# ChristophReich1996/Multi-StyleGAN

Measured on AMD Instinct MI355X. Metric: training images/sec (G+D step, 256^2, seq=3x2ch), higher is better.
Workload: dtype bf16

## Files before the change

### include/msg_hip.h

```cpp
#ifndef MSG_HIP_H
#define MSG_HIP_H

#ifdef __cplusplus
extern "C" {
#endif

enum { MSG_OK = 0, MSG_EINVAL = -1, MSG_EUNSUPPORTED = -2, MSG_ELAUNCH = -3 };
enum { MSG_F32 = 0, MSG_BF16 = 1, MSG_F16 = 2, MSG_F64 = 3, MSG_F32_SPLIT = 4 };

#define MSG_ABI_VERSION 5
int msg_abi_version(void);
const char* msg_build_arch(void);
const char* msg_strerror(int code);

int msg_upfirdn2d(const void* x, const float* fir, void* y, int dtype,
                  int major, int in_h, int in_w, int minor, int kh, int kw,
                  int up_x, int up_y, int down_x, int down_y,
                  int pad_x0, int pad_x1, int pad_y0, int pad_y1, void* stream);

int msg_upfirdn2d_pitched(const void* x, const float* fir, void* y, int dtype,
                          int major, int in_h, int in_w, int minor, int in_pitch, int kh, int kw,
                          int up_x, int up_y, int down_x, int down_y,
                          int pad_x0, int pad_x1, int pad_y0, int pad_y1, void* stream);

int msg_upfirdn2d_pitched2(const void* x, const float* fir, void* y, int dtype,
                           int major, int in_h, int in_w, int minor, int in_pitch, int out_pitch, int kh, int kw,
                           int up_x, int up_y, int down_x, int down_y,
                           int pad_x0, int pad_x1, int pad_y0, int pad_y1, void* stream);

int msg_upfirdn2d_separable(const void* x, const float* fir_y, const float* fir_x, void* y, int dtype,
                            int major, int in_h, int in_w, int minor, int kh, int kw,
                            int pad_x0, int pad_x1, int pad_y0, int pad_y1, void* stream);

int msg_upfirdn2d_separable_act(const void* x, const float* fir_y, const float* fir_x, void* y, int dtype,
                                int major, int in_h, int in_w, int minor, int kh, int kw,
                                int pad_x0, int pad_x1, int pad_y0, int pad_y1,
                                const float* act_bias, const float* noise, const float* noise_weight,
                                int noise_batch, float alpha, float scale, void* stream);
int msg_upfirdn2d_separable_act_mask(const void* x, const float* fir_y, const float* fir_x, void* y, int dtype,
                                     int major, int in_h, int in_w, int minor, int kh, int kw,
                                     int pad_x0, int pad_x1, int pad_y0, int pad_y1,
                                     const float* act_bias, const float* noise, const float* noise_weight,
                                     int noise_batch, float alpha, float scale, unsigned char* mask, void* stream);

int msg_fused_bias_act(const void* x, const float* bias, const void* ref, void* y, int dtype,
                       long long size_x, int step_b, int size_b,
                       const float* noise, const float* noise_weight, int noise_batch, int pix,
                       int act, int grad, float alpha, float scale, void* stream);

long long msg_bias_act_backward_workspace(long long size_x, int step_b, int size_b, int has_noise);
int msg_bias_act_backward(const void* gy, const void* out, void* gx, int dtype,
                          long long size_x, int step_b, int size_b,
                          float* grad_bias, const float* noise, float* grad_noise_weight,
                          int noise_batch, int pix, float alpha, float scale,
                          float* ws, long long ws_floats, void* stream);
int msg_channel_sums(const void* x, float* sums, int dtype, long long size_x, int C, float* ws, long long ws_floats,
                     void* stream);
int msg_bias_act_backward_mask(const void* gy, const unsigned char* mask, int tile_m, int tile_n, void* gx, int dtype,
                               long long size_x, int size_b,
                               float* grad_bias, const float* noise, float* grad_noise_weight,
                               int noise_batch, int pix, float alpha, float scale,
                               float* ws, long long ws_floats, void* stream);
int msg_sum_rows(const float* part, float* out, long long rows, int cols, void* stream);
int msg_bias_act_backward_mask_head(const void* gy, const void* ghead, const float* whead, const float* style,
                                    float wscale, int n_head, const unsigned char* mask, int tile_m, int tile_n,
                                    void* gx, int dtype, long long size_x, int size_b,
                                    float* grad_bias, const float* noise, float* grad_noise_weight,
                                    int noise_batch, int pix, float alpha, float scale,
                                    float* ws, long long ws_floats, void* stream);

int msg_conv2d_fprop(const void* x, const void* w, const float* bias, void* y, int dtype,
                     int B, int IH, int IW, int Cx, int Ck, int OH, int OW, int N, int ldy,
                     int kh, int kw, int stride, int pad, int in_up, int pixel_shuffle,
                     long long w_batch_stride, void* stream);
enum { MSG_WGRAD_K_AUTO = -1 };
int msg_conv2d_wgrad(const void* gy, const void* x, float* gw, int dtype,
                     int B, int IH, int IW, int Cx, int I, int OH, int OW, int ldgy, int O, int ldgw,
                     int kh, int kw, int stride, int pad, int pixel_shuffle,
                     int per_sample, int k_chunks, int oi_major, float gain,
                     float* ws, long long ws_floats, void* stream);
long long msg_conv2d_wgrad_workspace(int dtype, int B, int IH, int IW, int Cx, int I, int OH, int OW, int ldgy,
                                     int O, int ldgw, int kh, int kw, int stride, int pad, int pixel_shuffle,
                                     int per_sample, int k_chunks);

int msg_demod_coeff(const float* W, const float* s, float* d, int B, int O, int I, int taps,
                    float scale, float eps, void* stream);
int msg_scale_rows_cols(const float* base, const float* rowscale, const float* colscale, void* out,
                        int dtype, int B, int R, int T, int C, int Ck, float gain, void* stream);
int msg_modulate_weights(const float* base, const float* wsq, const float* style, void* out, float* d_out,
                         int dtype, int B, int R, int O, int T, int C, int Ck, float scale, float eps, void* stream);
int msg_modulate_backward(const float* gwk, const float* W, const float* s, const float* d, float* gW,
                          float* gs_part, int B, int O, int I, int taps, int ldg, int o_group,
                          float scale, void* stream);
int msg_scale_rows_cols2(const float* base, const float* row1, const float* col1, const float* row2, const float* col2,
                         void* out, int dtype, int B, int R, int T, int C, int Ck, float gain, void* stream);
int msg_modulate_backward2(const float* gwk, const float* W, const float* s, const float* d, const float* v,
                           float* gW, float* gs_part, int B, int O, int I, int taps, int ldg, int o_group,
                           float scale, void* stream);

int msg_relayout_weight(const float* w, void* fwd, void* dgrad, float* wsq, int dtype,
                        int O, int I, int T, int Ck, int Ok, int flip, int t_major, float gain, void* stream);

int msg_gather_taps(const void* x, void* y, int dtype, int B, int H, int W, int Cx, int C, int kh, int kw,
                    int pad, int Ko, void* stream);
int msg_fold_taps(const void* g, const void* add, void* gx, int dtype, int B, int H, int W, int Ko, int C, int kh, int kw,
                  int pad, int ldx, int ld_add, void* stream);

int msg_scaled_add(const void* a, const void* b, void* y, int dtype, long long n, float beta, float gain, void* stream);
int msg_rgb_skip_merge(const void* conv, int dtype, int ld, const float* bias, const float* skip, const float* fir,
                       float* out, int B, int C, int H, int W, void* stream);
int msg_rgb_skip_merge_backward(const float* g, void* g_conv, int dtype, int ld, float* g_skip, const float* fir,
                                int B, int C, int H, int W, void* stream);
int msg_gamma_merge(const void* a, const void* b, const float* gamma, void* y, int dtype, long long n, float gain, void* stream);
long long msg_gamma_merge_backward_workspace(void);
int msg_gamma_merge_backward(const void* gy, const void* a, const float* gamma, void* ga, void* gb, float* g_gamma, int dtype,
                             long long n, float gain, float* ws, void* stream);
int msg_scaled_add_rows(const void* a, const void* b, void* y, int dtype, long long rows, int cols,
                        long long lda, long long ldb, long long ldy, float beta, float gain, void* stream);

int msg_softmax_rows(const void* x, void* y, int dtype, long long rows, int cols, void* stream);
int msg_softmax_rows_backward(const void* y, const void* gy, void* gx, int dtype, long long rows, int cols,
                              void* stream);
int msg_softmax_rows_backward2(const void* y, const void* gy, const void* v, void* d_y, void* d_gy, int dtype,
                               long long rows, int cols, void* stream);

int msg_nonlocal_attention_supported(int B, int Nq, int Nk, int dk, int dv);
int msg_nonlocal_attention_fwd(const void* q, const void* k, const void* vt, void* o, float* lse, int dtype,
                               int B, int Nq, int Nk, int dk, int dv, void* stream);
int msg_maxpool2x2_fwd(const void* x, void* y, unsigned short* idx, int dtype, int B, int H, int W, int C, long long ldx,
                       void* stream);
int msg_maxpool2x2_bwd(const void* gy, const unsigned short* idx, void* gx, int dtype, int B, int H, int W, int C,
                       void* stream);
int msg_maxpool2x2_gather(const void* v, const unsigned short* idx, void* out, int dtype, int B, int H, int W, int C,
                          long long ldv, void* stream);

int msg_nonlocal_attention_bwd_splits(int B, int Nq, int Nk);
int msg_nonlocal_attention_bwd(const void* q, const void* qt, const void* k, const void* kt, const void* v,
                               const void* dO, const void* dOt, const void* o, const float* lse, float* delta,
                               void* dq, void* dk_out, void* dv_out, float* workspace, int dtype,
                               int B, int Nq, int Nk, int dk, int dv, void* stream);

int msg_affine_warp(const float* x, float* y, const float* angle_deg, float angle_const, const float* scale_xy,
                    const float* select_u, const float* p, int rot_prob, float cx, float cy, int padding,
                    int align_corners, int B, int C, int H, int W, int backward, void* workspace, void* stream);

long long msg_minibatch_stddev_workspace(int C, int H, int W, int groups, int dtype);
int msg_minibatch_stddev(const void* x, void* y, float* stat, float* workspace, int dtype,
                         int B, int C, int H, int W, int ldx, int ldy, int groups, float alpha, void* stream);
int msg_minibatch_stddev_backward(const void* x, const void* gy, const float* gstat, void* gx, int dtype,
                                  int B, int C, int H, int W, int ldx, int ldgy, int ldgx, int groups,
                                  float alpha, void* stream);

int msg_conv2d_fprop_act(const void* x, const void* w, void* y, int dtype,
                         int B, int IH, int IW, int Cx, int Ck, int OH, int OW, int N, int ldy,
                         int kh, int kw, int stride, int pad, long long w_batch_stride,
                         const float* act_bias, const float* noise, const float* noise_weight,
                         int noise_batch, float alpha, float scale, void* stream);
int msg_conv2d_fprop_act_mask(const void* x, const void* w, void* y, int dtype,
                              int B, int IH, int IW, int Cx, int Ck, int OH, int OW, int N, int ldy,
                              int kh, int kw, int stride, int pad, long long w_batch_stride,
                              const float* act_bias, const float* noise, const float* noise_weight,
                              int noise_batch, float alpha, float scale, unsigned char* mask, void* stream);

int msg_conv2d_fprop_residual(const void* x, const void* w, void* y, int dtype,
                              int B, int IH, int IW, int Cx, int Ck, int OH, int OW, int N, int ldy,
                              int kh, int kw, int stride, int pad, long long w_batch_stride,
                              const void* residual, int res_ld, float gain, void* stream);

int msg_conv2d_fprop_act_backward(const void* x, const void* w, void* y, int dtype,
                                  int B, int IH, int IW, int Cx, int Ck, int OH, int OW, int N, int ldy,
                                  int kh, int kw, int stride, int pad, long long w_batch_stride,
                                  const void* residual, int res_ld,
                                  const unsigned char* sign_mask, int mask_tile_m, int mask_tile_n,
                                  const void* sign_map, int sign_ld, float alpha, float scale,
                                  float* grad_bias, const float* noise, int noise_batch, float* grad_noise_weight,
                                  float* ws, long long ws_floats, void* stream);

int msg_act_pointwise_head(const void* x, const float* bias, const float* w, float* y, int dtype,
                           long long npix, int C, float wscale, float alpha, float scale, void* stream);
long long msg_act_pointwise_head_backward_workspace(long long npix, int C);
int msg_act_pointwise_head_backward(const void* x, const float* bias, const float* w, const float* gy, void* gx,
// ... 111 lines not shown
```

### multi_stylegan_amd/conv_ops.py

```python
import ctypes
import functools
import math
import os
from typing import Optional, Tuple

import torch
from torch.autograd import Function

from . import _lib, weight_images
from ._autograd import _derive
from .weight_images import _k_run, _oi, _round_up
from .weight_images import invalidate_weight_cache


def _vec(dtype) -> int:
    return 8 if dtype == torch.bfloat16 else 4


def _padded_nhwc(b, c, h, w, dtype, device):
    cx = _round_up(c, _vec(dtype))
    buf = torch.empty((b, h, w, cx), dtype=dtype, device=device)
    if cx != c:
        buf[..., c:].zero_()
    return buf.permute(0, 3, 1, 2)[:, :c]
# ... 1250 lines not shown
        if not terms:
            return (None, None, None, None)
        grads = torch.autograd.grad(sum(terms), leaves, allow_unused=True)
    return tuple(gr if w else None for gr, w in zip(grads, want))


class _ModConvGrad(Function):

    @staticmethod
    def forward(ctx, gy, x, weight, style, d, demodulate, upsample, g, scale, need):
        gx, gw, gs, gwk = _modconv_backward(x, weight, style, d, gy, demodulate, upsample, g, scale, need, keep_gwk=True)
        ctx.set_materialize_grads(False)
        ctx.save_for_backward(gy, x, weight, style, d, gwk)
        ctx.cfg = (demodulate, upsample, g, scale)
        return gx, gw, gs

    @staticmethod
    @torch.autograd.function.once_differentiable
    def backward(ctx, a, cot_w, cot_s):
        gy, x, weight, style, d, gwk = ctx.saved_tensors
        demodulate, upsample, g, scale = ctx.cfg
        want = ctx.needs_input_grad[:4]
        _, o, i, kh, kw = weight.shape
        b, t = x.shape[0], kh * kw
        tail = (None,) * 6
        if a is None and cot_w is None and cot_s is None:
            return (None, None, None, None) + tail
        if cot_w is not None or i % 4 or i > 512 or t not in (1, 4, 9) or b > _MODCONV_BWD_BATCH or \
                (cot_s is not None and gwk is None):
            return _modconv_second_order_composite(gy, x, weight, style, demodulate, upsample, a, cot_w, cot_s, want) + tail
        dev = x.device
        w3 = weight.detach().reshape(o, i, t)
        s = style.detach().float().contiguous()
        dd = d if demodulate else None
        ck, okp = _round_up(i, _k_run(gy.dtype)), _round_up(o, _k_run(gy.dtype))
        rows = t * o if upsample else o
        ggy = gx2 = gw3 = gs2 = None
        if a is not None:
            a = a.to(x.dtype)
            if want[0]:
                wk = torch.empty((b, rows, 1 if upsample else t, ck), dtype=x.dtype, device=dev)
                base = weight_images.forward(weight, torch.float32, 1.0, g.kind, modulation=True)[0]
                _scale_rows_cols(base, (d.repeat(1, t) if upsample else d) if demodulate else None, s, wk, scale)
                ggy = _f_image(a, wk, ck, o, i, g)
            if want[2] or want[3]:
                gwk_a, ldg = _g_raw(gy, a, o, i, g, raw=True)
                gw3, gs2 = _fold_weight_gradient(gwk_a, ldg, w3, s, dd, scale, style.dtype)
        if cot_s is not None:
            v = cot_s.detach().float().contiguous()
            if want[0] or want[1]:
                hf = torch.empty((b, rows, 1 if upsample else t, ck), dtype=x.dtype, device=dev)
                hd = torch.empty((b, i, t, okp), dtype=gy.dtype, device=dev)
                base_f = weight_images.forward(weight, torch.float32, 1.0, g.kind, modulation=True)[0]
                base_d = weight_images.dgrad(weight, torch.float32, 1.0, g.kind, modulation=True)[0]
                if demodulate:
                    wsq = weight_images.tap_square_sums(weight, g.kind)
                    ddir = -(scale * scale) * d.pow(3) * linear(s * v, wsq)
                    rows_d, rows_dd = (d.repeat(1, t), ddir.repeat(1, t)) if upsample else (d, ddir)
                    with _lib.on_device(dev):
                        lib, st = _lib.lib(), _lib.stream_of(dev)
                        code = lib.msg_scale_rows_cols2(base_f.data_ptr(), rows_d.contiguous().data_ptr(), v.data_ptr(),
                                                        rows_dd.contiguous().data_ptr(), s.data_ptr(), hf.data_ptr(),
                                                        _lib.dtype_code(hf), b, rows, 1 if upsample else t, i, ck, scale, st)
                        _lib.check(code, "msg_scale_rows_cols2")
                        code = lib.msg_scale_rows_cols2(base_d.data_ptr(), v.data_ptr(), d.data_ptr(), s.data_ptr(),
                                                        ddir.contiguous().data_ptr(), hd.data_ptr(), _lib.dtype_code(hd), b, i, t,
                                                        o, okp, scale, st)
                        _lib.check(code, "msg_scale_rows_cols2")
                else:
                    _scale_rows_cols(base_f, None, v, hf, scale)
                    _scale_rows_cols(base_d, v, None, hd, scale)
                if want[0]:
                    ggy = _f_image(x, hf, ck, o, i, g, residual=None if ggy is None else (ggy, 1.0))
                if want[1]:
                    gx2 = _d_image(gy, hd, okp, o, i, g)
            if want[2] or want[3]:
                gw3b, gs2b = _fold_weight_gradient(gwk, gwk.shape[-1], w3, s, dd, scale, style.dtype, cotangent=v)
                gw3 = gw3b if gw3 is None else gw3 + gw3b
                gs2 = gs2b if gs2 is None else gs2 + gs2b
        gw = gw3.reshape(1, o, i, kh, kw) if (gw3 is not None and want[2]) else None
        return (ggy, gx2, gw, gs2 if want[3] else None) + tail


class _ModulatedConv(Function):

    @staticmethod
    def forward(ctx, x, weight, style, demodulate, upsample, act_bias=None, noise=None, noise_w=None, alpha=0.2,
                act_scale=1.0, fuse_act=False, head_slot=None, input_act=None):
        dev = _lib.require_gpu(x, weight, style)
        ctx.input_act = input_act if input_act is not None and input_act.armed else None
        ctx.head_slot = head_slot
        if head_slot is not None and fuse_act:
            ctx.set_materialize_grads(False)
            head_slot.armed = True
        _, o, i, kh, kw = weight.shape
        b, t = x.shape[0], kh * kw
        scale = math.sqrt(2.0) / math.sqrt(i * t)
        s = style.detach().float().contiguous()
        d = None
        ck = _round_up(i, _k_run(x.dtype))
        kind = "up2" if upsample else "conv"
        base = weight_images.forward(weight, torch.float32, 1.0, kind, modulation=True)[0]
        rows = t * o if upsample else o
        wk = torch.empty((b, rows, 1 if upsample else t, ck), dtype=x.dtype, device=dev)
        if demodulate:
            wsq = weight_images.tap_square_sums(weight, kind)
            d = torch.empty((b, o), dtype=torch.float32, device=dev)
            with _lib.on_device(dev):
                code = _lib.lib().msg_modulate_weights(base.data_ptr(), wsq.data_ptr(), s.data_ptr(), wk.data_ptr(),
                                                       d.data_ptr(), _lib.dtype_code(wk), b, rows, o,
                                                       1 if upsample else t, i, ck, scale, 1e-8, _lib.stream_of(dev))
            _lib.check(code, "msg_modulate_weights")
        else:
            _scale_rows_cols(base, None, s, wk, scale)
        g = Geometry(kind, kh, kw, 1, kh // 2, x.shape[2:], True)
        act = None
        holder = [] if any(ctx.needs_input_grad) else None
        if fuse_act:
            assert not upsample, "the upsampling layers blur before their activation"
            act = (*_act_operands(act_bias, noise, noise_w, (b, o, *g.y_hw)), alpha, act_scale, holder)
        y = _f_image(x, wk, ck, o, i, g, act=act)
        ctx.save_for_backward(x, weight, style, d if d is not None else torch.empty(0, device=dev),
                              y if fuse_act else None, noise if fuse_act else None)
        ctx.cfg = (demodulate, upsample, g, scale)
        ctx.act = (alpha, act_scale, act_bias is not None, noise is not None,
                   None if noise_w is None else noise_w.shape) if fuse_act else None
        ctx.bias_param = act_bias
        ctx.mask = holder[0] if holder else None
        return y

    @staticmethod
    def backward(ctx, gy):
        x, weight, style, d, y_act, noise = ctx.saved_tensors
        demodulate, upsample, g, scale = ctx.cfg
        _, o, i, kh, kw = weight.shape
        b, t = x.shape[0], kh * kw
        need = list(ctx.needs_input_grad)
        need[1], need[2] = _consumed(ctx, 1, 1), _consumed(ctx, 2, 2)
        gb = gnw = None
        slot = ctx.head_slot
        if ctx.act is not None:
            from .op_static.fused_act import FusedLeakyReLUFunctionBackward, act_backward_with_head
            alpha, act_scale, has_bias, has_noise, nw_shape = ctx.act
            head, head_dgrad = slot.take() if slot is not None else (None, None)
            fused = None
            if head is not None:
                fused = act_backward_with_head(gy, head, y_act.shape, noise if has_noise else None,
                                               ctx.bias_param if has_bias else None, has_bias, alpha, act_scale, ctx.mask)
                if fused is None:
                    gh = head_dgrad()
                    gy = gh if gy is None else gy + gh
            if fused is not None:
                gy, gb, gnw = fused
            elif gy is None:
                return (None,) * 13
            else:
                gy, gb, gnw = _derive(FusedLeakyReLUFunctionBackward, gy, y_act, noise if has_noise else None,
                                      ctx.bias_param if has_bias else False, alpha, act_scale, ctx.mask)
            gb = gb if has_bias and need[5] else None
            gnw = gnw.reshape(nw_shape) if has_noise and need[7] else None
        tail = (None, None, gb, None, gnw, None, None, None, None, None)
        if ctx.act is None and slot is not None and slot.armed and need[0] and not torch.is_grad_enabled() and \
                fused_head_ok(gy, weight, b, demodulate, upsample):
            gyc, wt, st = gy, weight, style
            slot.head = (gyc, weight.detach().reshape(o, i).float().contiguous(), style.detach().float().contiguous(), scale)
            slot.dgrad = lambda: _modconv_backward(x, wt, st, d, gyc, demodulate, upsample, g, scale,
                                                   [True, False, False])[0]
            need[0] = False
        fused_ok = i <= 512 and t <= 9
        if torch.is_grad_enabled() and fused_ok and _NATIVE_SECOND_ORDER and b <= _MODCONV_BWD_BATCH and x.is_cuda:
            gx, gw, gs = _derive(_ModConvGrad, gy, x, weight, style, d if demodulate else None, demodulate, upsample, g, scale,
                                            tuple(need[:3]))
            return (gx, gw, gs) + tail
        if torch.is_grad_enabled() or not fused_ok:
            with torch.enable_grad():
                ins = [v for v, n in zip((x, weight, style), need[:3]) if n]
                y2 = _modulated_composite(x, weight, style, demodulate, upsample)
                grads = list(torch.autograd.grad(y2, ins, gy, create_graph=torch.is_grad_enabled(), allow_unused=True))
            out = [grads.pop(0) if n else None for n in need[:3]]
            return (out[0], out[1], out[2]) + tail
        if b > _MODCONV_BWD_BATCH:
            gxs, gws, gss = [], [], []
            for lo in range(0, b, _MODCONV_BWD_BATCH):
                hi = min(b, lo + _MODCONV_BWD_BATCH)
                cgx, cgw, cgs = _modconv_backward(x[lo:hi], weight, style[lo:hi], d[lo:hi] if demodulate else d,
                                                  gy[lo:hi], demodulate, upsample, g, scale, need)
                gxs.append(cgx); gws.append(cgw); gss.append(cgs)
            gx = torch.cat(gxs) if need[0] else None
            gw = torch.stack(gws).sum(dim=0) if gws[0] is not None else None
            gs = torch.cat(gss) if gss[0] is not None else None
            return (gx, gw, gs) + tail
        gx, gw, gs = _modconv_backward(x, weight, style, d, gy, demodulate, upsample, g, scale, need, direct=True,
                                       act_bwd=ctx.input_act)
        return (gx, gw, gs) + tail


def fused_head_ok(gy, weight, b, demodulate, upsample) -> bool:
    _, o, _, kh, kw = weight.shape
    return gy is not None and gy.is_cuda and gy.dtype == torch.bfloat16 and kh == 1 and kw == 1 and o <= 8 and \
        not demodulate and not upsample and b <= _MODCONV_BWD_BATCH and HEAD_GRAD_FUSION


HEAD_GRAD_FUSION = bool(int(os.environ.get("MSG_HEAD_GRAD_FUSION", "1")))

# ... 13 lines not shown
```

### multi_stylegan_amd/csrc/modulate.hip

```cpp
#include "msg_common.h"
#include <stdlib.h>

__device__ __forceinline__ float block_sum_256(float v, float* red ) {
    v = wave_sum(v);
    __syncthreads();
    if ((threadIdx.x & 63) == 0) red[threadIdx.x >> 6] = v;
    __syncthreads();
    return red[0] + red[1] + red[2] + red[3];
}

__global__ __launch_bounds__(256) void demod_coeff_kernel(const float* __restrict__ W, const float* __restrict__ s,
                                                          float* __restrict__ d, int B, int O, int I, int T,
                                                          float scale, float eps) {
    __shared__ float red[4];
    const int o = blockIdx.x;
    const float* wo = W + (size_t)o * I * T;
    for (int b = 0; b < B; ++b) {
        float acc = 0.f;
        for (int i = threadIdx.x; i < I; i += 256) {
            const float sv = s[(size_t)b * I + i];
            float w2 = 0.f;
            for (int t = 0; t < T; ++t) { const float wv = wo[i * T + t]; w2 = fmaf(wv, wv, w2); }
            acc = fmaf(w2, sv * sv, acc);
        }
        const float tot = block_sum_256(acc, red);
        if (threadIdx.x == 0) d[(size_t)b * O + o] = rsqrtf(scale * scale * tot + eps);
    }
}

extern "C" int msg_demod_coeff(const float* W, const float* s, float* d, int B, int O, int I, int taps,
                               float scale, float eps, void* stream) {
    if (B == 0) return MSG_OK;
    if (!W || !s || !d || B < 0 || O <= 0 || I <= 0 || taps <= 0) return MSG_EINVAL;
    hipLaunchKernelGGL(demod_coeff_kernel, dim3(O), dim3(256), 0, (hipStream_t)stream, W, s, d, B, O, I, taps, scale, eps);
    return MSG_CHECK_LAUNCH();
}

template <int VEC>
__device__ __forceinline__ void load_run(const float* __restrict__ src, int c0, int limit, bool aligned, float (&f)[VEC]) {
    if (aligned && c0 + VEC <= limit) {
#pragma unroll
        for (int e = 0; e < VEC; e += 4) {
            const float4 v = *reinterpret_cast<const float4*>(src + c0 + e);
            f[e] = v.x; f[e + 1] = v.y; f[e + 2] = v.z; f[e + 3] = v.w;
        }
    } else {
#pragma unroll
        for (int e = 0; e < VEC; ++e) f[e] = (c0 + e < limit) ? src[c0 + e] : 0.f;
    }
}

constexpr int SRC_ITEMS = 5;
template <typename TO>
__global__ __launch_bounds__(256) void scale_rows_cols_kernel(const float* __restrict__ base,
                                                              const float* __restrict__ rowscale,
                                                              const float* __restrict__ colscale, TO* __restrict__ out,
                                                              int B, int BG, int R, int T, int C, int Ck, float gain) {
    using V = Vec16<TO>;
    constexpr int VEC = V::N;
    const int r = blockIdx.x, b0 = blockIdx.y * BG, b1 = min(B, b0 + BG);
    const int cvecs = Ck / VEC;
    const float* src_row = base + (size_t)r * T * C;
    const int tstep = 256 / cvecs > 0 ? 256 / cvecs : 1;
    const bool al = (C % 4 == 0) && ((((uintptr_t)base | (uintptr_t)colscale) & 15u) == 0);
    for (int cv = threadIdx.x % cvecs; cv < cvecs; cv += 256) {
        const int c0 = cv * VEC;
        const int t0 = threadIdx.x / cvecs;
        for (int tb = t0; tb < T; tb += tstep * SRC_ITEMS) {
            float f[SRC_ITEMS][VEC];
#pragma unroll
            for (int k = 0; k < SRC_ITEMS; ++k) {
                const int t = tb + k * tstep;
                if (t < T) load_run<VEC>(src_row + (size_t)t * C, c0, C, al, f[k]);
                else {
#pragma unroll
                    for (int e = 0; e < VEC; ++e) f[k][e] = 0.f;
                }
            }
            for (int b = b0; b < b1; ++b) {
                const float rs = gain * (rowscale ? rowscale[(size_t)b * R + r] : 1.f);
                float sc[VEC];
                if (colscale) load_run<VEC>(colscale + (size_t)b * C, c0, C, al, sc);
                else {
// ... 49 lines not shown
                                                               TO* __restrict__ out, int B, int BG, int R, int T, int C, int Ck,
                                                               float gain) {
    using V = Vec16<TO>;
    constexpr int VEC = V::N;
    const int r = blockIdx.x, b0 = blockIdx.y * BG, b1 = min(B, b0 + BG);
    const int cvecs = Ck / VEC;
    const float* src_row = base + (size_t)r * T * C;
    const int tstep = 256 / cvecs > 0 ? 256 / cvecs : 1;
    const bool al = (C % 4 == 0) && ((((uintptr_t)base | (uintptr_t)col1 | (uintptr_t)col2) & 15u) == 0);
    for (int cv = threadIdx.x % cvecs; cv < cvecs; cv += 256) {
        const int c0 = cv * VEC;
        const int t0 = threadIdx.x / cvecs;
        for (int tb = t0; tb < T; tb += tstep * SRC_ITEMS) {
            float f[SRC_ITEMS][VEC];
#pragma unroll
            for (int k = 0; k < SRC_ITEMS; ++k) {
                const int t = tb + k * tstep;
                if (t < T) load_run<VEC>(src_row + (size_t)t * C, c0, C, al, f[k]);
                else {
#pragma unroll
                    for (int e = 0; e < VEC; ++e) f[k][e] = 0.f;
                }
            }
            for (int b = b0; b < b1; ++b) {
                const float rs1 = gain * row1[(size_t)b * R + r], rs2 = gain * row2[(size_t)b * R + r];
                float sc[VEC], s2[VEC];
                load_run<VEC>(col1 + (size_t)b * C, c0, C, al, sc);
                load_run<VEC>(col2 + (size_t)b * C, c0, C, al, s2);
#pragma unroll
                for (int e = 0; e < VEC; ++e) sc[e] = fmaf(rs1, sc[e], rs2 * s2[e]);
                TO* dst_row = out + ((size_t)b * R + r) * T * Ck;
#pragma unroll
                for (int k = 0; k < SRC_ITEMS; ++k) {
                    const int t = tb + k * tstep;
                    if (t >= T) break;
                    V o;
                    if constexpr (VEC == 4) {
#pragma unroll
                        for (int e = 0; e < 4; ++e) o.set(e, f[k][e] * sc[e]);
                    } else {
#pragma unroll
                        for (int e = 0; e < 4; ++e) o.set2(e, f[k][2 * e] * sc[2 * e], f[k][2 * e + 1] * sc[2 * e + 1]);
                    }
                    *reinterpret_cast<uint4*>(dst_row + (size_t)t * Ck + c0) = o.raw;
                }
            }
        }
    }
}

extern "C" int msg_scale_rows_cols2(const float* base, const float* row1, const float* col1, const float* row2,
                                    const float* col2, void* out, int dtype, int B, int R, int T, int C, int Ck, float gain,
                                    void* stream) {
    if (B == 0) return MSG_OK;
    if (!base || !row1 || !col1 || !row2 || !col2 || !out || B < 0 || R <= 0 || T <= 0 || C <= 0 || Ck < C) return MSG_EINVAL;
    if (dtype != MSG_F32 && dtype != MSG_BF16) return MSG_EUNSUPPORTED;
    const int vec = dtype == MSG_BF16 ? 8 : 4;
    if (Ck % vec || (((uintptr_t)out) & 15u)) return MSG_EUNSUPPORTED;
    hipStream_t s = (hipStream_t)stream;
    int bg = 1;
    while (bg < 8 && bg * 2 <= B && (long long)R * ((B + 2 * bg - 1) / (2 * bg)) >= 2048) bg *= 2;
    dim3 grid(R, (B + bg - 1) / bg);
    if (dtype == MSG_BF16)
        hipLaunchKernelGGL((scale_rows_cols2_kernel<bf16_t>), grid, dim3(256), 0, s, base, row1, col1, row2, col2,
                           (bf16_t*)out, B, bg, R, T, C, Ck, gain);
    else
        hipLaunchKernelGGL((scale_rows_cols2_kernel<float>), grid, dim3(256), 0, s, base, row1, col1, row2, col2,
                           (float*)out, B, bg, R, T, C, Ck, gain);
    return MSG_CHECK_LAUNCH();
}

template <typename TO>
__global__ __launch_bounds__(256) void modulate_weights_kernel(const float* __restrict__ base, const float* __restrict__ wsq,
                                                               const float* __restrict__ style, TO* __restrict__ out,
                                                               float* __restrict__ d_out, int B, int BG, int R, int O,
                                                               int T, int C, int Ck, float scale, float eps) {
    using V = Vec16<TO>;
    constexpr int VEC = V::N;
    __shared__ float red[4 * 8];
    __shared__ float dsh[8];
    const int o = blockIdx.x, b0 = blockIdx.y * BG, b1 = min(B, b0 + BG);
    {
        float part[8];
#pragma unroll
        for (int k = 0; k < 8; ++k) part[k] = 0.f;
        for (int i = threadIdx.x; i < C; i += 256) {
            const float q = wsq[(size_t)o * C + i];
#pragma unroll
            for (int k = 0; k < 8; ++k)
                if (b0 + k < b1) { const float sv = style[(size_t)(b0 + k) * C + i]; part[k] = fmaf(q, sv * sv, part[k]); }
        }
#pragma unroll
        for (int k = 0; k < 8; ++k) {
            const float v = wave_sum(part[k]);
            if ((threadIdx.x & 63) == 0) red[(threadIdx.x >> 6) * 8 + k] = v;
        }
        __syncthreads();
        if (threadIdx.x < 8 && b0 + (int)threadIdx.x < b1) {
            const int k = threadIdx.x;
            const float tot = red[k] + red[8 + k] + red[16 + k] + red[24 + k];
            const float dv = rsqrtf(scale * scale * tot + eps);
            dsh[k] = dv;
            if (d_out) d_out[(size_t)(b0 + k) * O + o] = dv;
        }
        __syncthreads();
    }
    const int cvecs = Ck / VEC;
    const int tstep = 256 / cvecs > 0 ? 256 / cvecs : 1;
    const bool al = (C % 4 == 0) && ((((uintptr_t)base | (uintptr_t)style) & 15u) == 0);
    const int npairs = (R / O) * T;
    for (int cv = threadIdx.x % cvecs; cv < cvecs; cv += 256) {
        const int c0 = cv * VEC;
        const int t0 = threadIdx.x / cvecs;
        for (int qb = t0; qb < npairs; qb += tstep * SRC_ITEMS) {
            float f[SRC_ITEMS][VEC];
            size_t cell[SRC_ITEMS];
#pragma unroll
            for (int k = 0; k < SRC_ITEMS; ++k) {
                const int q = qb + k * tstep;
                const int rk = q / T, t = q - rk * T;
                cell[k] = (size_t)(o + rk * O) * T + t;
                if (q < npairs) load_run<VEC>(base + cell[k] * C, c0, C, al, f[k]);
                else {
#pragma unroll
                    for (int e = 0; e < VEC; ++e) f[k][e] = 0.f;
                }
            }
            for (int b = b0; b < b1; ++b) {
                const float rs = scale * dsh[b - b0];
                float sc[VEC];
                load_run<VEC>(style + (size_t)b * C, c0, C, al, sc);
#pragma unroll
                for (int e = 0; e < VEC; ++e) sc[e] *= rs;
                TO* dst_b = out + (size_t)b * R * T * Ck;
#pragma unroll
                for (int k = 0; k < SRC_ITEMS; ++k) {
                    if (qb + k * tstep >= npairs) break;
                    V ov;
                    if constexpr (VEC == 4) {
#pragma unroll
                        for (int e = 0; e < 4; ++e) ov.set(e, f[k][e] * sc[e]);
                    } else {
#pragma unroll
                        for (int e = 0; e < 4; ++e) ov.set2(e, f[k][2 * e] * sc[2 * e], f[k][2 * e + 1] * sc[2 * e + 1]);
                    }
                    *reinterpret_cast<uint4*>(dst_b + cell[k] * Ck + c0) = ov.raw;
                }
            }
        }
    }
}

extern "C" int msg_modulate_weights(const float* base, const float* wsq, const float* style, void* out, float* d_out,
                                    int dtype, int B, int R, int O, int T, int C, int Ck, float scale, float eps,
                                    void* stream) {
    if (B == 0) return MSG_OK;
    if (!base || !wsq || !style || !out || B < 0 || R <= 0 || O <= 0 || R % O || T <= 0 || C <= 0 || Ck < C) return MSG_EINVAL;
    if (dtype != MSG_F32 && dtype != MSG_BF16) return MSG_EUNSUPPORTED;
    const int vec = dtype == MSG_BF16 ? 8 : 4;
    if (Ck % vec || ((uintptr_t)out & 15u) || B > 65535) return MSG_EUNSUPPORTED;
    hipStream_t s = (hipStream_t)stream;
    static const int min_wgs = msg_tunable("MSG_MODW_MIN_WGS", 1024);
    int bg = 1;
    while (bg < 8 && bg * 2 <= B && (long long)O * ((B + 2 * bg - 1) / (2 * bg)) >= min_wgs) bg *= 2;
    dim3 grid(O, (B + bg - 1) / bg);
    if (dtype == MSG_BF16)
        hipLaunchKernelGGL((modulate_weights_kernel<bf16_t>), grid, dim3(256), 0, s, base, wsq, style, (bf16_t*)out, d_out,
                           B, bg, R, O, T, C, Ck, scale, eps);
    else
        hipLaunchKernelGGL((modulate_weights_kernel<float>), grid, dim3(256), 0, s, base, wsq, style, (float*)out, d_out,
                           B, bg, R, O, T, C, Ck, scale, eps);
    return MSG_CHECK_LAUNCH();
}

constexpr int MB_SLOTS = 2;
constexpr int MB_TAPS = 9;
constexpr int MB_BMAX = 32;
template <bool DEMOD>
__global__ __launch_bounds__(256) void modulate_backward_kernel(const float* __restrict__ gwk, const float* __restrict__ W,
                                                                const float* __restrict__ s, const float* __restrict__ d,
                                                                float* __restrict__ gW, float* __restrict__ gs_part,
                                                                int B, int O, int I, int T, int ldg, int OG, float scale) {
    __shared__ float red[4 * MB_BMAX];
    __shared__ float Tsh[MB_BMAX];
// ... 423 lines not shown
```

Measured before the change: 157.0.

## Fuse weight modulation, demodulation and conv into one kernel for small resolutions

```diff
diff --git a/include/msg_hip.h b/include/msg_hip.h
--- a/include/msg_hip.h
+++ b/include/msg_hip.h
@@ -97,6 +97,12 @@
 int msg_modulate_backward2(const float* gwk, const float* W, const float* s, const float* d, const float* v,
                            float* gW, float* gs_part, int B, int O, int I, int taps, int ldg, int o_group,
                            float scale, void* stream);
+enum { MSG_MODCONV_CONV3 = 0, MSG_MODCONV_UP2 = 1 };
+int msg_modconv2d_small_fprop(const void* x, const float* base, const float* wsq, const float* style, void* y,
+                              float* d_out, int dtype, int B, int H, int W, int Cx, int I, int O, int kind, int ldy,
+                              float scale, float eps, int demodulate, int fuse_act, const float* act_bias,
+                              const float* noise, const float* noise_weight, int noise_batch, float alpha,
+                              float act_scale, unsigned char* sign_mask, void* stream);
 
 int msg_relayout_weight(const float* w, void* fwd, void* dgrad, float* wsq, int dtype,
                         int O, int I, int T, int Ck, int Ok, int flip, int t_major, float gain, void* stream);
diff --git a/multi_stylegan_amd/conv_ops.py b/multi_stylegan_amd/conv_ops.py
--- a/multi_stylegan_amd/conv_ops.py
+++ b/multi_stylegan_amd/conv_ops.py
@@ -1356,6 +1356,38 @@
         return (ggy, gx2, gw, gs2 if want[3] else None) + tail
 
 
+_SMALL_MODCONV = True
+_small_modconv_code = None
+_SMALL_MODCONV_PIXELS = {"conv": 64, "up2": 16}
+
+
+def _modconv_small(x, base, wsq, s, o, i, g: Geometry, scale, act):
+    global _small_modconv_code
+    dev = x.device
+    xv, cx = _nhwc_view(x)
+    b, _, h, w_ = xv.shape
+    up2 = g.kind == "up2"
+    y, ldy = _alloc_out(b, o, 2 * h, 2 * w_, x.dtype, dev) if up2 else _alloc_out(b, o, h, w_, x.dtype, dev)
+    d = torch.empty((b, o), dtype=torch.float32, device=dev) if wsq is not None else None
+    act_bias, noise, noise_w, alpha, act_scale = act[:5] if act is not None else (None, None, None, 0.0, 1.0)
+    key = "conv_fprop_modsmall"
+    if _lib.kernel_clock.enabled and _CLOCK_SHAPES:
+        key += _shape_key(b, (h, w_), g.y_hw if not up2 else (h, w_), i, 4 * o if up2 else o, 1 if up2 else 3, 1 if up2 else 3, 1,
+                          " up1 ps per-sample" if up2 else " up1 per-sample")
+    flops = 2.0 * b * h * w_ * o * i * (4 if up2 else 9)
+    with _lib.on_device(dev), _lib.kernel_clock.span((key, 'bf16'), flops):
+        code = _lib.lib().msg_modconv2d_small_fprop(
+            xv.data_ptr(), base.data_ptr(), _lib.ptr(wsq), s.data_ptr(), y.data_ptr(), _lib.ptr(d), _lib.dtype_code(x), b, h, w_,
+            cx, i, o, _lib.MSG_MODCONV_UP2 if up2 else _lib.MSG_MODCONV_CONV3, ldy, scale, 1e-8, int(wsq is not None),
+            int(act is not None), _lib.ptr(act_bias), _lib.ptr(noise), _lib.ptr(noise_w), 1 if noise is None else noise.shape[0],
+            float(alpha), float(act_scale), None, _lib.stream_of(dev))
+    _small_modconv_code = code
+    if code == _lib.MSG_EUNSUPPORTED:
+        return None, None
+    _lib.check(code, "msg_modconv2d_small_fprop")
+    return y, d
+
+
 class _ModulatedConv(Function):
 
     @staticmethod
@@ -1376,24 +1408,29 @@
         kind = "up2" if upsample else "conv"
         base = weight_images.forward(weight, torch.float32, 1.0, kind, modulation=True)[0]
         rows = t * o if upsample else o
-        wk = torch.empty((b, rows, 1 if upsample else t, ck), dtype=x.dtype, device=dev)
-        if demodulate:
-            wsq = weight_images.tap_square_sums(weight, kind)
-            d = torch.empty((b, o), dtype=torch.float32, device=dev)
-            with _lib.on_device(dev):
-                code = _lib.lib().msg_modulate_weights(base.data_ptr(), wsq.data_ptr(), s.data_ptr(), wk.data_ptr(),
-                                                       d.data_ptr(), _lib.dtype_code(wk), b, rows, o,
-                                                       1 if upsample else t, i, ck, scale, 1e-8, _lib.stream_of(dev))
-            _lib.check(code, "msg_modulate_weights")
-        else:
-            _scale_rows_cols(base, None, s, wk, scale)
         g = Geometry(kind, kh, kw, 1, kh // 2, x.shape[2:], True)
         act = None
         holder = [] if any(ctx.needs_input_grad) else None
         if fuse_act:
             assert not upsample, "the upsampling layers blur before their activation"
             act = (*_act_operands(act_bias, noise, noise_w, (b, o, *g.y_hw)), alpha, act_scale, holder)
-        y = _f_image(x, wk, ck, o, i, g, act=act)
+        wsq = weight_images.tap_square_sums(weight, kind) if demodulate else None
+        y = None
+        if _SMALL_MODCONV and x.dtype == torch.bfloat16 and x.shape[2] * x.shape[3] <= _SMALL_MODCONV_PIXELS[kind] and \
+                ((kh, kw) == (2, 2) if upsample else (kh, kw) == (3, 3)):
+            y, d = _modconv_small(x, base, wsq, s, o, i, g, scale, act)
+        if y is None:
+            wk = torch.empty((b, rows, 1 if upsample else t, ck), dtype=x.dtype, device=dev)
+            if demodulate:
+                d = torch.empty((b, o), dtype=torch.float32, device=dev)
+                with _lib.on_device(dev):
+                    code = _lib.lib().msg_modulate_weights(base.data_ptr(), wsq.data_ptr(), s.data_ptr(), wk.data_ptr(),
+                                                           d.data_ptr(), _lib.dtype_code(wk), b, rows, o,
+                                                           1 if upsample else t, i, ck, scale, 1e-8, _lib.stream_of(dev))
+                _lib.check(code, "msg_modulate_weights")
+            else:
+                _scale_rows_cols(base, None, s, wk, scale)
+            y = _f_image(x, wk, ck, o, i, g, act=act)
         ctx.save_for_backward(x, weight, style, d if d is not None else torch.empty(0, device=dev),
                               y if fuse_act else None, noise if fuse_act else None)
         ctx.cfg = (demodulate, upsample, g, scale)
diff --git a/multi_stylegan_amd/csrc/modconv_small.hip b/multi_stylegan_amd/csrc/modconv_small.hip
--- /dev/null
+++ b/multi_stylegan_amd/csrc/modconv_small.hip
@@ -0,0 +1,314 @@
+#include "msg_common.h"
+#include "modulate_demod.h"
+
+typedef __bf16 bf16v8 __attribute__((ext_vector_type(8)));
+typedef const __attribute__((address_space(1))) f32x4* gf4_t;
+
+struct ModConvParams {
+    int B, H, W, Cx, C, Ck, O, N, T, ldy;
+    int up2, demod;
+    int rows_per_tile, m_tiles, n_slices, xcd_slices;
+    int a_pitch;
+    float scale, eps;
+    long long x_bstride, y_bstride;
+    ActEpilogue act;
+};
+
+constexpr int MC_RING = 8;
+constexpr int MC_MAX_TILE = 128;
+constexpr int MC_LDS = 160 * 1024;
+constexpr int MC_WROW = 144;
+
+__host__ __device__ inline int mc_fixed_lds(int Ck, int NS, int a_pitch) {
+    return Ck * 4 + NS * 4 + 4 * NS * 4 + 2 * NS * MC_WROW + a_pitch;
+}
+
+template <int NS>
+__global__ __launch_bounds__(256, 1) void modconv_small_kernel(const bf16_t* __restrict__ x, const float* __restrict__ base,
+                                                               const float* __restrict__ wsq, const float* __restrict__ style,
+                                                               bf16_t* __restrict__ y, float* __restrict__ d_out, ModConvParams p) {
+    constexpr int CB = NS / 32;
+    constexpr int GROUPS = 4 / CB;
+    constexpr int PBW = (MC_MAX_TILE / 32) / GROUPS;
+    extern __shared__ __attribute__((aligned(16))) char smem[];
+    float* sty = reinterpret_cast<float*>(smem);
+    float* dsh = sty + p.Ck;
+    float* red = dsh + NS;
+    char* wbuf = reinterpret_cast<char*>(red + 4 * NS);
+    char* zrow = wbuf + 2 * NS * MC_WROW;
+    char* aimg = zrow + p.a_pitch;
+
+    const int tid = threadIdx.x, lane = tid & 63, wid = tid >> 6;
+    const int lr = lane & 31, lh = lane >> 5;
+    int slice, rem;
+    {
+        const int per_slice = p.m_tiles * p.B;
+        if (p.xcd_slices) {
+            const int xcd = blockIdx.x & 7, k = blockIdx.x >> 3;
+            const int j = k / per_slice;
+            rem = k - j * per_slice;
+            slice = xcd + 8 * j;
+        } else {
+            slice = blockIdx.x / per_slice;
+            rem = blockIdx.x - slice * per_slice;
+        }
+    }
+    const int b = rem / p.m_tiles, tile = rem - b * p.m_tiles;
+    const int n0 = slice * NS;
+    const int r0 = tile * p.rows_per_tile, r1 = min(p.H, r0 + p.rows_per_tile);
+    const int lo = p.up2 ? r0 : max(r0 - 1, 0), hi = p.up2 ? r1 : min(p.H, r1 + 1);
+    const int mt = (r1 - r0) * p.W;
+    const int C = p.C, Ck = p.Ck;
+
+    for (int c = tid; c < Ck; c += 256) sty[c] = c < C ? style[(size_t)b * C + c] : 0.f;
+    if (p.demod) {
+#pragma unroll
+        for (int c32 = 0; c32 < NS; c32 += 32) {
+            size_t wrow[32], srow[32];
+#pragma unroll
+            for (int k = 0; k < 32; ++k) {
+                const int n = n0 + c32 + k;
+                wrow[k] = (size_t)(n < p.N ? n % p.O : 0) * C;
+                srow[k] = (size_t)b * C;
+            }
+            float part[32];
+            demod_wave_partials<32>(wsq, style, wrow, srow, 32, C, tid, part);
+#pragma unroll
+            for (int k = 0; k < 32; ++k)
+                if (lane == 0) red[wid * NS + c32 + k] = part[k];
+        }
+        __syncthreads();
+        if (tid < NS) {
+            const float dv = demod_from_wave_sums(red[tid], red[NS + tid], red[2 * NS + tid], red[3 * NS + tid], p.scale, p.eps);
+            dsh[tid] = p.scale * dv;
+            const int n = n0 + tid;
+            if (d_out && tile == 0 && n < p.O) d_out[(size_t)b * p.O + n] = dv;
+        }
+    } else if (tid < NS) {
+        dsh[tid] = p.scale;
+    }
+    {
+        const int vecs = Ck >> 3, total = (hi - lo) * p.W * vecs;
+        const bf16_t* xb = x + (long long)b * p.x_bstride + (long long)lo * p.W * p.Cx;
+        for (int v = tid; v < total; v += 256) {
+            const int pix = v / vecs, c = (v - pix * vecs) << 3;
+            u32x4 val = {0u, 0u, 0u, 0u};
+            if (c < p.Cx) val = *reinterpret_cast<const u32x4*>(xb + (long long)pix * p.Cx + c);
+            *reinterpret_cast<u32x4*>(aimg + pix * p.a_pitch + c * 2) = val;
+        }
+        for (int v = tid; v < (p.a_pitch >> 4); v += 256) *reinterpret_cast<u32x4*>(zrow + v * 16) = u32x4{0u, 0u, 0u, 0u};
+    }
+    __syncthreads();
+
+    const int cb = wid % CB, grp = wid / CB;
+    const bool wave_on = n0 + 32 * cb < p.N && 32 * grp < mt;
+    int a_oh[PBW], a_ow[PBW];
+    bool a_in[PBW], pb_on[PBW];
+#pragma unroll
+    for (int i = 0; i < PBW; ++i) {
+        const int m = 32 * (grp + GROUPS * i) + lr;
+        pb_on[i] = wave_on && 32 * (grp + GROUPS * i) < mt;
+        a_in[i] = m < mt;
+        const int mm = a_in[i] ? m : 0;
+        a_oh[i] = r0 + mm / p.W;
+        a_ow[i] = mm % p.W;
+    }
+    f32x16 acc[PBW];
+#pragma unroll
+    for (int i = 0; i < PBW; ++i)
+#pragma unroll
+        for (int e = 0; e < 16; ++e) acc[i][e] = 0.f;
+
+    constexpr int LPT = NS / 16;
+    const int wr = tid >> 4, wv = tid & 15;
+    const float* wrowp[LPT];
+    float rsj[LPT];
+#pragma unroll
+    for (int j = 0; j < LPT; ++j) {
+        wrowp[j] = base + (size_t)min(n0 + wr + 16 * j, p.N - 1) * p.T * C;
+        rsj[j] = dsh[wr + 16 * j];
+    }
+    const int n_chunks = Ck >> 6, n_iters = p.T * n_chunks;
+    const int pad = p.up2 ? 0 : 1;
+    f32x4 ring[MC_RING][LPT];
+    int lq = 0, l_tap = 0, l_ch = 0;
+    auto request = [&](f32x4 (&dst)[LPT]) __attribute__((always_inline)) {
+        const size_t off = (size_t)l_tap * C + min(l_ch * 64 + 4 * wv, C - 4);
+#pragma unroll
+        for (int j = 0; j < LPT; ++j) dst[j] = *(gf4_t)(wrowp[j] + off);
+        if (lq + 1 < n_iters) {
+            ++lq;
+            if (++l_ch == n_chunks) { l_ch = 0; ++l_tap; }
+        }
+    };
+    int v_ch = 0;
+    auto convert = [&](const f32x4 (&src)[LPT], char* wb) __attribute__((always_inline)) {
+        const int c = v_ch * 64 + 4 * wv;
+        const bool live = c < C;
+        const f32x4 s4 = *reinterpret_cast<const f32x4*>(sty + c);
+#pragma unroll
+        for (int j = 0; j < LPT; ++j) {
+            float f[4], sc[4];
+#pragma unroll
+            for (int e = 0; e < 4; ++e) {
+                f[e] = live ? src[j][e] : 0.f;
+                sc[e] = s4[e];
+            }
+#pragma unroll
+            for (int e = 0; e < 4; ++e) sc[e] *= rsj[j];
+            uint2 pk;
+            pk.x = (uint32_t)f2bf(f[0] * sc[0]) | ((uint32_t)f2bf(f[1] * sc[1]) << 16);
+            pk.y = (uint32_t)f2bf(f[2] * sc[2]) | ((uint32_t)f2bf(f[3] * sc[3]) << 16);
+            *reinterpret_cast<uint2*>(wb + (wr + 16 * j) * MC_WROW + wv * 8) = pk;
+        }
+        if (++v_ch == n_chunks) v_ch = 0;
+    };
+    int c_tap = 0, c_ch = 0;
+    auto contract = [&](const char* wb) __attribute__((always_inline)) {
+        if (wave_on) {
+            const int kh = p.up2 ? 0 : c_tap / 3, kw = p.up2 ? 0 : c_tap - 3 * kh;
+            const char* ap[PBW];
+#pragma unroll
+            for (int i = 0; i < PBW; ++i) {
+                const int ih = a_oh[i] + kh - pad, iw = a_ow[i] + kw - pad;
+                const bool ok = a_in[i] & ((unsigned)ih < (unsigned)p.H) & ((unsigned)iw < (unsigned)p.W);
+                ap[i] = (ok ? aimg + ((ih - lo) * p.W + iw) * p.a_pitch : zrow) + c_ch * 128;
+            }
+            const char* wp = wb + (32 * cb + lr) * MC_WROW;
+#pragma unroll
+            for (int kk = 0; kk < 4; ++kk) {
+                const int ko = (kk * 16 + lh * 8) * 2;
+                const bf16v8 wf = *reinterpret_cast<const bf16v8*>(wp + ko);
+#pragma unroll
+                for (int i = 0; i < PBW; ++i) {
+                    if (!pb_on[i]) continue;
+                    const bf16v8 af = *reinterpret_cast<const bf16v8*>(ap[i] + ko);
+                    acc[i] = __builtin_amdgcn_mfma_f32_32x32x16_bf16(wf, af, acc[i], 0, 0, 0);
+                }
+            }
+        }
+        if (++c_ch == n_chunks) { c_ch = 0; ++c_tap; }
+    };
+#pragma unroll
+    for (int r = 0; r < MC_RING; ++r) request(ring[r]);
+    convert(ring[0], wbuf);
+    request(ring[0]);
+    for (int q0 = 0; q0 < n_iters; q0 += MC_RING) {
+#pragma unroll
+        for (int r = 0; r < MC_RING; ++r) {
+            if (q0 + r >= n_iters) break;
+            __syncthreads();
+            if (q0 + r + 1 < n_iters) convert(ring[(r + 1) % MC_RING], wbuf + ((r + 1) & 1) * NS * MC_WROW);
+            request(ring[(r + 1) % MC_RING]);
+            contract(wbuf + (r & 1) * NS * MC_WROW);
+        }
+    }
+    if (!wave_on) return;
+
+    const int hw = p.H * p.W;
+    const bool act_on = p.act.enabled == 1;
+    const bool want_noise = act_on && p.act.noise;
+    const float nw = want_noise ? p.act.noise_w[0] : 0.f;
+    bf16_t* yb = y + (long long)b * p.y_bstride;
+#pragma unroll
+    for (int i = 0; i < PBW; ++i) {
+        if (!pb_on[i] || !a_in[i]) continue;
+        const int pix = a_oh[i] * p.W + a_ow[i];
+        const float nv = want_noise ? nw * p.act.noise[(long long)(p.act.noise_batch == 1 ? 0 : b) * hw + pix] : 0.f;
+#pragma unroll
+        for (int g = 0; g < 4; ++g) {
+            const int n4 = n0 + 32 * cb + 8 * g + 4 * lh;
+            if (n4 >= p.N) continue;
+            uint2 pk;
+            pk.x = (unsigned)f2bf(acc[i][4 * g + 0] + 0.f) | ((unsigned)f2bf(acc[i][4 * g + 1] + 0.f) << 16);
+            pk.y = (unsigned)f2bf(acc[i][4 * g + 2] + 0.f) | ((unsigned)f2bf(acc[i][4 * g + 3] + 0.f) << 16);
+            if (act_on) {
+                float bv[8];
+#pragma unroll
+                for (int e = 0; e < 8; ++e) bv[e] = (p.act.bias && e < 4 && n4 + e < p.N) ? p.act.bias[n4 + e] : 0.f;
+                const u32x4 r = act_epilogue_apply<bf16_t>(u32x4{pk.x, pk.y, 0u, 0u}, bv, nv, p.act.alpha, p.act.scale);
+                pk.x = r[0]; pk.y = r[1];
+            }
+            long long opix = pix;
+            int c = n4;
+            if (p.up2) {
+                const int q = n4 / p.O;
+                c = n4 - q * p.O;
+                opix = (long long)(2 * a_oh[i] + (q >> 1)) * (2 * p.W) + 2 * a_ow[i] + (q & 1);
+            }
+            bf16_t* dst = yb + opix * p.ldy + c;
+            if (n4 + 4 <= p.N) {
+                *reinterpret_cast<uint2*>(dst) = pk;
+            } else {
+                const unsigned w[2] = {pk.x, pk.y};
+                for (int e = 0; e < p.N - n4; ++e) dst[e] = (bf16_t)(w[e >> 1] >> (16 * (e & 1)));
+            }
+        }
+    }
+}
+
+static int mc_rows_per_tile(int H, int W, int halo, int a_pitch, int fixed) {
+    int rows = 0;
+    for (int r = 1; r <= H; ++r) {
+        const long long held = (long long)std::min(H, r + halo) * W * a_pitch;
+        if ((long long)r * W > MC_MAX_TILE || fixed + held > MC_LDS) break;
+        rows = r;
+    }
+    if (!rows) return 0;
+    const int tiles = (H + rows - 1) / rows;
+    return (H + tiles - 1) / tiles;
+}
+
+template <int NS>
+static int mc_launch(const ModConvParams& p0, const void* x, const float* base, const float* wsq, const float* style, void* y,
+                     float* d_out, hipStream_t st) {
+    ModConvParams p = p0;
+    const int fixed = mc_fixed_lds(p.Ck, NS, p.a_pitch);
+    p.rows_per_tile = mc_rows_per_tile(p.H, p.W, p.up2 ? 0 : 2, p.a_pitch, fixed);
+    if (!p.rows_per_tile) return MSG_EUNSUPPORTED;
+    p.m_tiles = (p.H + p.rows_per_tile - 1) / p.rows_per_tile;
+    p.n_slices = (p.N + NS - 1) / NS;
+    p.xcd_slices = p.n_slices % 8 == 0;
+    const long long blocks = (long long)p.n_slices * p.m_tiles * p.B;
+    if (blocks >= (1ll << 31)) return MSG_EUNSUPPORTED;
+    const int held = std::min(p.H, p.rows_per_tile + (p.up2 ? 0 : 2)) * p.W;
+    const int lds = fixed + held * p.a_pitch;
+    static const hipError_t attr = hipFuncSetAttribute(reinterpret_cast<const void*>(&modconv_small_kernel<NS>),
+                                                       hipFuncAttributeMaxDynamicSharedMemorySize, MC_LDS);
+    if (attr != hipSuccess) return MSG_ELAUNCH;
+    hipLaunchKernelGGL((modconv_small_kernel<NS>), dim3((unsigned)blocks), dim3(256), lds, st, (const bf16_t*)x, base, wsq, style,
+                       (bf16_t*)y, d_out, p);
+    return MSG_CHECK_LAUNCH();
+}
+
+extern "C" int msg_modconv2d_small_fprop(const void* x, const float* base, const float* wsq, const float* style, void* y,
+                                         float* d_out, int dtype, int B, int H, int W, int Cx, int I, int O, int kind, int ldy,
+                                         float scale, float eps, int demodulate, int fuse_act, const float* act_bias,
+                                         const float* noise, const float* noise_weight, int noise_batch, float alpha,
+                                         float act_scale, unsigned char* sign_mask, void* stream) {
+    if (B == 0) return MSG_OK;
+    if (!x || !base || !style || !y || B < 0 || H <= 0 || W <= 0 || Cx <= 0 || I <= 0 || I > Cx || O <= 0 || ldy < O ||
+        (kind != MSG_MODCONV_CONV3 && kind != MSG_MODCONV_UP2) || (demodulate && !wsq))
+        return MSG_EINVAL;
+    if (fuse_act && noise && (!noise_weight || (noise_batch != 1 && noise_batch != B))) return MSG_EINVAL;
+    if (dtype != MSG_BF16 || (long long)H * W > 256 || Cx % 8 || I % 8 || ldy % 8) return MSG_EUNSUPPORTED;
+    if (kind == MSG_MODCONV_UP2 && (O % 8 || fuse_act)) return MSG_EUNSUPPORTED;
+    if (sign_mask) return MSG_EUNSUPPORTED;
+    if ((((uintptr_t)x | (uintptr_t)base | (uintptr_t)style | (uintptr_t)y) & 15u) || B > 65535) return MSG_EUNSUPPORTED;
+    ModConvParams p{};
+    p.B = B; p.H = H; p.W = W; p.Cx = Cx; p.C = I; p.Ck = (I + 63) / 64 * 64; p.O = O; p.ldy = ldy;
+    p.up2 = kind == MSG_MODCONV_UP2;
+    p.N = p.up2 ? 4 * O : O;
+    p.T = p.up2 ? 1 : 9;
+    p.demod = demodulate != 0;
+    p.a_pitch = p.Ck * 2 + 16;
+    p.scale = scale; p.eps = eps;
+    p.x_bstride = (long long)H * W * Cx;
+    p.y_bstride = (p.up2 ? 4ll : 1ll) * H * W * ldy;
+    if (p.Ck > 4096) return MSG_EUNSUPPORTED;
+    if (fuse_act) p.act = ActEpilogue{act_bias, noise, noise_weight, noise_batch, 1, alpha, act_scale, nullptr, 0, 0.f, nullptr};
+    static const int forced = msg_tunable("MSG_MODCONV_NS", 0);
+    const bool wide = forced ? forced == 64 : (long long)H * W > 64;
+    return wide ? mc_launch<64>(p, x, base, wsq, style, y, d_out, (hipStream_t)stream)
+                : mc_launch<32>(p, x, base, wsq, style, y, d_out, (hipStream_t)stream);
+}
diff --git a/multi_stylegan_amd/csrc/modulate.hip b/multi_stylegan_amd/csrc/modulate.hip
--- a/multi_stylegan_amd/csrc/modulate.hip
+++ b/multi_stylegan_amd/csrc/modulate.hip
@@ -1,4 +1,5 @@
 #include "msg_common.h"
+#include "modulate_demod.h"
 #include <stdlib.h>
 
 __device__ __forceinline__ float block_sum_256(float v, float* red ) {
@@ -214,24 +215,17 @@
     const int o = blockIdx.x, b0 = blockIdx.y * BG, b1 = min(B, b0 + BG);
     {
         float part[8];
-#pragma unroll
-        for (int k = 0; k < 8; ++k) part[k] = 0.f;
-        for (int i = threadIdx.x; i < C; i += 256) {
-            const float q = wsq[(size_t)o * C + i];
-#pragma unroll
-            for (int k = 0; k < 8; ++k)
-                if (b0 + k < b1) { const float sv = style[(size_t)(b0 + k) * C + i]; part[k] = fmaf(q, sv * sv, part[k]); }
-        }
-#pragma unroll
-        for (int k = 0; k < 8; ++k) {
-            const float v = wave_sum(part[k]);
-            if ((threadIdx.x & 63) == 0) red[(threadIdx.x >> 6) * 8 + k] = v;
-        }
+        size_t wrow[8], srow[8];
+#pragma unroll
+        for (int k = 0; k < 8; ++k) { wrow[k] = (size_t)o * C; srow[k] = (size_t)(b0 + k) * C; }
+        demod_wave_partials<8>(wsq, style, wrow, srow, b1 - b0, C, threadIdx.x, part);
+#pragma unroll
+        for (int k = 0; k < 8; ++k)
+            if ((threadIdx.x & 63) == 0) red[(threadIdx.x >> 6) * 8 + k] = part[k];
         __syncthreads();
         if (threadIdx.x < 8 && b0 + (int)threadIdx.x < b1) {
             const int k = threadIdx.x;
-            const float tot = red[k] + red[8 + k] + red[16 + k] + red[24 + k];
-            const float dv = rsqrtf(scale * scale * tot + eps);
+            const float dv = demod_from_wave_sums(red[k], red[8 + k], red[16 + k], red[24 + k], scale, eps);
             dsh[k] = dv;
             if (d_out) d_out[(size_t)(b0 + k) * O + o] = dv;
         }
diff --git a/multi_stylegan_amd/csrc/modulate_demod.h b/multi_stylegan_amd/csrc/modulate_demod.h
--- /dev/null
+++ b/multi_stylegan_amd/csrc/modulate_demod.h
@@ -0,0 +1,27 @@
+#pragma once
+#include "msg_common.h"
+
+template <int K>
+__device__ __forceinline__ void demod_wave_partials(const float* __restrict__ wsq, const float* __restrict__ style,
+                                                    const size_t (&wrow)[K], const size_t (&srow)[K], int nk, int C, int first,
+                                                    float (&out)[K]) {
+    float part[K];
+#pragma unroll
+    for (int k = 0; k < K; ++k) part[k] = 0.f;
+    for (int i = first; i < C; i += 256) {
+#pragma unroll
+        for (int k = 0; k < K; ++k)
+            if (k < nk) {
+                const float q = wsq[wrow[k] + i];
+                const float sv = style[srow[k] + i];
+                part[k] = fmaf(q, sv * sv, part[k]);
+            }
+    }
+#pragma unroll
+    for (int k = 0; k < K; ++k) out[k] = wave_sum(part[k]);
+}
+
+__device__ __forceinline__ float demod_from_wave_sums(float r0, float r1, float r2, float r3, float scale, float eps) {
+    const float tot = r0 + r1 + r2 + r3;
+    return rsqrtf(scale * scale * tot + eps);
+}
```

Result: no change. 157.4, median of 6 (+0.2%).
